# taichi-dev/taichi-nerfs

Measured on AMD Instinct MI355X. Metric: training rays/sec, higher is better.
Workload: dtype f32-table+f16-mlp

## Files before the change

taichi-nerfs_amd/csrc/mlp.hip:

```cpp
#include "ngp_device.h"
#include <stdlib.h>

namespace ngp {

typedef _Float16 half_t;
typedef half_t half8 __attribute__((ext_vector_type(8)));
typedef half_t half4 __attribute__((ext_vector_type(4)));
typedef float floatx4 __attribute__((ext_vector_type(4)));

#define NGP_MFMA(a, b, c) __builtin_amdgcn_mfma_f32_16x16x32_f16((a), (b), (c), 0, 0, 0)

constexpr int N_FWD_FRAGS = 20;
constexpr int N_ALL_FRAGS = 42;
constexpr int F_W1 = 0;
constexpr int F_W2 = 4;
constexpr int F_W3 = 6;
constexpr int F_W4 = 10;
constexpr int F_W5 = 18;
constexpr int B_W5T = 20;
constexpr int B_W4T = 24;
constexpr int B_W3T = 32;
constexpr int B_W2T = 34;
constexpr int B_W1T = 38;

__device__ __forceinline__ int chain_k(int s, int g, int j) { return 32 * s + 16 * (j >> 2) + 4 * g + (j & 3); }

__device__ __forceinline__ int pair_nat(int p, int slot) { return slot < 2 ? 2 * p + slot : 2 * (15 - p) + (slot - 2); }
__device__ __forceinline__ int enc_feat(int pairs, int g, int j) { return pairs ? pair_nat(2 * g + (j >> 2), j & 3) : 8 * g + j; }
__device__ __forceinline__ int enc_row(int pairs, int mt, int i) { return pairs ? pair_nat(4 * mt + (i >> 2), i & 3) : 16 * mt + i; }

__device__ __forceinline__ void pack_one(int tid, const float* W1, const float* W2, const float* W3, const float* W4,
                                         const float* W5, int pairs, half_t* wpack) {
    const int j = tid & 7, lane = (tid >> 3) & 63, frag = tid >> 9;
    const int i = lane & 15, g = lane >> 4;
    float v = 0.0f;
    if (frag < F_W2) {
        const int mt = frag - F_W1;
        v = W1[(16 * mt + i) * 32 + enc_feat(pairs, g, j)];
    } else if (frag < F_W3) {
        const int s = frag - F_W2;
        v = W2[i * 64 + chain_k(s, g, j)];
    } else if (frag < F_W4) {
        const int mt = frag - F_W3;
        const int k = (j < 4) ? (4 * g + j) : (16 + 4 * g + (j - 4));
        v = W3[(16 * mt + i) * 32 + k];
    } else if (frag < F_W5) {
        const int mt = (frag - F_W4) >> 1, s = (frag - F_W4) & 1;
        v = W4[(16 * mt + i) * 64 + chain_k(s, g, j)];
    } else if (frag < B_W5T) {
        const int s = frag - F_W5;
        v = (i < 3) ? W5[i * 64 + chain_k(s, g, j)] : 0.0f;
    } else if (frag < B_W4T) {
        const int mt = frag - B_W5T;
        const int k = 4 * g + j;
        v = (j < 4 && k < 3) ? W5[k * 64 + 16 * mt + i] : 0.0f;
    } else if (frag < B_W3T) {
        const int mt = (frag - B_W4T) >> 1, s = (frag - B_W4T) & 1;
        v = W4[chain_k(s, g, j) * 64 + 16 * mt + i];
    } else if (frag < B_W2T) {
        const int s = frag - B_W3T;
        v = W3[chain_k(s, g, j) * 32 + 16 + i];
    } else if (frag < B_W1T) {
        const int mt = frag - B_W2T;
        v = (j < 4) ? W2[(4 * g + j) * 64 + 16 * mt + i] : 0.0f;
    } else {
        const int mt = (frag - B_W1T) >> 1, s = (frag - B_W1T) & 1;
        v = W1[chain_k(s, g, j) * 32 + enc_row(pairs, mt, i)];
    }
    wpack[tid] = (half_t)v;
}

__global__ void __launch_bounds__(256) mlp_pack_kernel(const float* __restrict__ W1, const float* __restrict__ W2,
                                                       const float* __restrict__ W3, const float* __restrict__ W4,
                                                       const float* __restrict__ W5, int pairs, half_t* __restrict__ wpack) {
    const int tid = blockIdx.x * blockDim.x + threadIdx.x;
    if (tid < N_ALL_FRAGS * 64 * 8) pack_one(tid, W1, W2, W3, W4, W5, pairs, wpack);
}

__device__ __forceinline__ void adam_mlp_pack_block(float* __restrict__ p, float* __restrict__ g, float* __restrict__ m,
                                                    float* __restrict__ v, const float* __restrict__ sf,
                                                    const int32_t* __restrict__ si, float beta1, float beta2, float eps,
                                                    int pairs, half_t* __restrict__ wpack) {
    __shared__ float wl[9408];
    const bool skip = si[SI_SKIP] != 0;
    const AdamConsts ac = adam_consts(sf, beta1, beta2, eps);
    constexpr int PER = (9408 + 1023) / 1024;
    float pi[PER], gi[PER], mi[PER], vi[PER];
#pragma unroll
    for (int k = 0; k < PER; ++k) {
        const int i = (int)threadIdx.x + 1024 * k, ic = i < 9408 ? i : 0;
        pi[k] = p[ic]; gi[k] = g[ic]; mi[k] = m[ic]; vi[k] = v[ic];
    }
#pragma unroll
    for (int k = 0; k < PER; ++k) {
        const int i = (int)threadIdx.x + 1024 * k;
        if (i >= 9408) continue;
        if (!skip) {
            float mk = mi[k], vk = vi[k];
            adam_update(pi[k], mk, vk, gi[k], ac);
            p[i] = pi[k]; m[i] = mk; v[i] = vk;
        }
        g[i] = 0.0f;
        wl[i] = pi[k];
    }
    __syncthreads();
    for (int item = threadIdx.x; item < N_ALL_FRAGS * 64; item += blockDim.x) {
#pragma unroll
        for (int j = 0; j < 8; ++j) pack_one(8 * item + j, wl, wl + 2048, wl + 3072, wl + 5120, wl + 9216, pairs, wpack);
    }
}

__global__ void __launch_bounds__(1024) adam_mlp_pack_kernel(float* __restrict__ p, float* __restrict__ g, float* __restrict__ m,
                                                             float* __restrict__ v, const float* __restrict__ sf,
                                                             const int32_t* __restrict__ si, float beta1, float beta2, float eps,
                                                             int pairs, half_t* __restrict__ wpack) {
    adam_mlp_pack_block(p, g, m, v, sf, si, beta1, beta2, eps, pairs, wpack);
}

template <int SHADOW, bool GRAD16>
__global__ void __launch_bounds__(1024) adam_all_kernel(float4* __restrict__ tp, void* __restrict__ tg, float4* __restrict__ tm,
                                                        float4* __restrict__ tv, long n4, uint2* __restrict__ shadow,
                                                        float* __restrict__ p, float* __restrict__ g, float* __restrict__ m,
                                                        float* __restrict__ v, const float* __restrict__ sf,
                                                        const int32_t* __restrict__ si, float beta1, float beta2, float eps,
                                                        int pairs, half_t* __restrict__ wpack) {
    if (blockIdx.x == 0) { if (p) adam_mlp_pack_block(p, g, m, v, sf, si, beta1, beta2, eps, pairs, wpack); }
    else adam_table_pass<SHADOW, GRAD16>(tp, tg, tm, tv, n4, sf, si, beta1, beta2, eps, shadow, (long)blockIdx.x - 1, (long)gridDim.x - 1);
}

typedef unsigned short ushort4v __attribute__((ext_vector_type(4)));
__device__ __forceinline__ half4 to_h4(const floatx4& d) { return __builtin_convertvector(d, half4); }
__device__ __forceinline__ half4 relu_h4(const floatx4& d) {
    const half4 z = {(half_t)0, (half_t)0, (half_t)0, (half_t)0};
    return __builtin_elementwise_max(to_h4(d), z);
}
__device__ __forceinline__ half8 cat_h4(const half4& a, const half4& b) {
    return __builtin_shufflevector(a, b, 0, 1, 2, 3, 4, 5, 6, 7);
}
__device__ __forceinline__ half4 mask_h4(const floatx4& d, const half4& act) {
    typedef unsigned int uint2v __attribute__((ext_vector_type(2)));
    const uint2v a = __builtin_bit_cast(uint2v, act), h = __builtin_bit_cast(uint2v, to_h4(d));
    uint2v r;
    asm("v_pk_sub_i16 %0, 0, %2\n\t"
        "v_pk_sub_i16 %1, 0, %3\n\t"
        "v_pk_ashrrev_i16 %0, 15, %0 op_sel_hi:[0,1]\n\t"
        "v_pk_ashrrev_i16 %1, 15, %1 op_sel_hi:[0,1]\n\t"
        "v_and_b32 %0, %0, %4\n\t"
        "v_and_b32 %1, %1, %5"
        : "=&v"(r.x), "=&v"(r.y) : "v"(a.x), "v"(a.y), "v"(h.x), "v"(h.y));
    return __builtin_bit_cast(half4, r);
}

__device__ __forceinline__ float fast_exp(float x) { return __expf(x); }
__device__ __forceinline__ float fast_rcp(float x) { return __builtin_amdgcn_rcpf(x); }
__device__ __forceinline__ float fast_rsq(float x) { return __builtin_amdgcn_rsqf(x); }

__device__ __forceinline__ half4 sh_quad(int g, float x, float y, float z) {
    const float xy = x * y, xz = x * z, yz = y * z, x2 = x * x, y2 = y * y, z2 = z * z;
    float a, b, c, d;
    if (g == 0) {
        a = 0.28209479177387814f; b = -0.48860251190291987f * y; c = 0.48860251190291987f * z; d = -0.48860251190291987f * x;
    } else if (g == 1) {
        a = 1.0925484305920792f * xy; b = -1.0925484305920792f * yz; c = 0.94617469575755997f * z2 - 0.31539156525251999f;
        d = -1.0925484305920792f * xz;
    } else if (g == 2) {
        a = 0.54627421529603959f * x2 - 0.54627421529603959f * y2; b = 0.59004358992664352f * y * (-3.0f * x2 + y2);
        c = 2.8906114426405538f * xy * z; d = 0.45704579946446572f * y * (1.0f - 5.0f * z2);
    } else {
        a = 0.3731763325901154f * z * (5.0f * z2 - 3.0f); b = 0.45704579946446572f * x * (1.0f - 5.0f * z2);
        c = 1.4453057213202769f * z * (x2 - y2); d = 0.59004358992664352f * x * (-x2 + 3.0f * y2);
    }
    half4 r;
    r[0] = (half_t)a; r[1] = (half_t)b; r[2] = (half_t)c; r[3] = (half_t)d;
    return r;
}

__device__ __forceinline__ half4 sh_quad_flat(int g, float x, float y, float z) {
    const float xy = x * y, xz = x * z, yz = y * z, x2 = x * x, y2 = y * y, z2 = z * z;
    const float a0 = 0.28209479177387814f, b0 = -0.48860251190291987f * y, c0 = 0.48860251190291987f * z, d0 = -0.48860251190291987f * x;
    const float a1 = 1.0925484305920792f * xy, b1 = -1.0925484305920792f * yz, c1 = 0.94617469575755997f * z2 - 0.31539156525251999f,
                d1 = -1.0925484305920792f * xz;
    const float a2 = 0.54627421529603959f * x2 - 0.54627421529603959f * y2, b2 = 0.59004358992664352f * y * (-3.0f * x2 + y2),
                c2 = 2.8906114426405538f * xy * z, d2 = 0.45704579946446572f * y * (1.0f - 5.0f * z2);
    const float a3 = 0.3731763325901154f * z * (5.0f * z2 - 3.0f), b3 = 0.45704579946446572f * x * (1.0f - 5.0f * z2),
                c3 = 1.4453057213202769f * z * (x2 - y2), d3 = 0.59004358992664352f * x * (-x2 + 3.0f * y2);
    const bool g0 = g == 0, g1 = g == 1, g2 = g == 2;
    half4 r;
    r[0] = (half_t)(g0 ? a0 : (g1 ? a1 : (g2 ? a2 : a3)));
    r[1] = (half_t)(g0 ? b0 : (g1 ? b1 : (g2 ? b2 : b3)));
    r[2] = (half_t)(g0 ? c0 : (g1 ? c1 : (g2 ? c2 : c3)));
    r[3] = (half_t)(g0 ? d0 : (g1 ? d1 : (g2 ? d2 : d3)));
    return r;
}

__device__ __forceinline__ void enc_ptrs(const float* __restrict__ enc, int pairs, size_t plane, int smp, int g, const float*& p0,
                                         const float*& p1) {
    if (pairs) { p0 = enc + ((size_t)(2 * g) * plane + smp) * 4; p1 = enc + ((size_t)(2 * g + 1) * plane + smp) * 4; }
    else { p0 = enc + (size_t)smp * 32 + 8 * g; p1 = p0 + 4; }
}

struct TileFwd {
    half8 b_enc;
    half4 a1[4];
    half4 h;
    half8 b_in3;
    half4 a3[4], a4[4];
    half4 rgb;
    float sigma;
};

__device__ __forceinline__ const half8& wfrag(const half8* __restrict__ wl, int id, int lane) { return wl[id * 64 + lane]; }

template <bool COLOR, bool FLAT_SH = false, class WF>
__device__ __forceinline__ void tile_forward_frags(const WF& W, int g, const float4& e0, const float4& e1,
                                                   float dx, float dy, float dz, TileFwd& t) {
    const floatx4 zero = {0.f, 0.f, 0.f, 0.f};
    t.b_enc[0] = (half_t)e0.x; t.b_enc[1] = (half_t)e0.y; t.b_enc[2] = (half_t)e0.z; t.b_enc[3] = (half_t)e0.w;
    t.b_enc[4] = (half_t)e1.x; t.b_enc[5] = (half_t)e1.y; t.b_enc[6] = (half_t)e1.z; t.b_enc[7] = (half_t)e1.w;
#pragma unroll
    for (int mt = 0; mt < 4; ++mt) t.a1[mt] = relu_h4(NGP_MFMA(W(F_W1 + mt), t.b_enc, zero));
    floatx4 d2 = NGP_MFMA(W(F_W2 + 0), cat_h4(t.a1[0], t.a1[1]), zero);
    d2 = NGP_MFMA(W(F_W2 + 1), cat_h4(t.a1[2], t.a1[3]), d2);
    t.h = to_h4(d2);
    t.sigma = expf((float)t.h[0]);
    if (!COLOR) return;
    const float inv = fast_rsq(dx * dx + dy * dy + dz * dz);
    const float x = (dx * inv + 1.0f) / 2.0f, y = (dy * inv + 1.0f) / 2.0f, z = (dz * inv + 1.0f) / 2.0f;
    t.b_in3 = cat_h4(FLAT_SH ? sh_quad_flat(g, x, y, z) : sh_quad(g, x, y, z), t.h);
    const float nan_dir = 0.0f * (x + y + z);
#pragma unroll
    for (int mt = 0; mt < 4; ++mt) t.a3[mt] = relu_h4(NGP_MFMA(W(F_W3 + mt), t.b_in3, zero));
    const half8 b30 = cat_h4(t.a3[0], t.a3[1]), b31 = cat_h4(t.a3[2], t.a3[3]);
#pragma unroll
    for (int mt = 0; mt < 4; ++mt) {
        floatx4 d4 = NGP_MFMA(W(F_W4 + 2 * mt), b30, zero);
        d4 = NGP_MFMA(W(F_W4 + 2 * mt + 1), b31, d4);
        t.a4[mt] = relu_h4(d4);
    }
    floatx4 d5 = NGP_MFMA(W(F_W5 + 0), cat_h4(t.a4[0], t.a4[1]), zero);
    d5 = NGP_MFMA(W(F_W5 + 1), cat_h4(t.a4[2], t.a4[3]), d5);
#pragma unroll
    for (int r = 0; r < 4; ++r) {
        const float c = (float)(half_t)d5[r] + nan_dir;
        t.rgb[r] = (half_t)fast_rcp(1.0f + fast_exp(-c));
    }
}

template <bool COLOR>
__device__ __forceinline__ void tile_forward_regs(const half8* __restrict__ wl, int lane, int g, const float4& e0, const float4& e1,
                                                  float dx, float dy, float dz, TileFwd& t) {
    tile_forward_frags<COLOR>([&](int id) -> const half8& { return wl[id * 64 + lane]; }, g, e0, e1, dx, dy, dz, t);
}

template <int THREADS, int N_FRAGS>
__device__ __forceinline__ void load_wpack(const half_t* __restrict__ wpack, half8* __restrict__ wl) {
    const uint4* src = reinterpret_cast<const uint4*>(wpack);
    uint4* dst = reinterpret_cast<uint4*>(wl);
    constexpr int PER = (N_FRAGS * 64 + THREADS - 1) / THREADS;
    uint4 v[PER];
#pragma unroll
    for (int i = 0; i < PER; ++i) {
        const int k = threadIdx.x + i * THREADS;
        v[i] = src[k < N_FRAGS * 64 ? k : 0];
    }
#pragma unroll
    for (int i = 0; i < PER; ++i) {
        const int k = threadIdx.x + i * THREADS;
        if (k < N_FRAGS * 64) dst[k] = v[i];
    }
    __syncthreads();
}

struct FwdIn { float4 e0, e1; float dx, dy, dz; };
template <bool COLOR, bool PAIRS>
__device__ __forceinline__ void fwd_request(FwdIn& raw, const float* __restrict__ enc, const float* __restrict__ dirs, int smp, int S,
                                            int g, size_t plane) {
    const size_t s0 = smp < S ? (size_t)smp : 0;
    const float *ep0, *ep1;
    enc_ptrs(enc, PAIRS ? 1 : 0, plane, (int)s0, g, ep0, ep1);
    raw.e0 = *reinterpret_cast<const float4*>(ep0);
// ... 213 lines not shown
            floatx4 dh = NGP_MFMA(wfrag(wl, B_W3T + 0, lane), cat_h4(dz3[0], dz3[1]), zero);
            dh = NGP_MFMA(wfrag(wl, B_W3T + 1, lane), cat_h4(dz3[2], dz3[3]), dh);
            dz2 = to_h4(dh);
            if (g == 0) {
                const float h0 = (float)t.h[0];
                const half_t gs = (half_t)(in.dsig * fast_exp(fminf(fmaxf(h0, -15.0f), 15.0f)));
                dz2[0] = (half_t)((float)dz2[0] + (float)gs);
            }
            __builtin_amdgcn_sched_barrier(0);
            const half8 b_dz2 = cat_h4(dz2, hzero);
#pragma unroll
            for (int mt = 0; mt < 4; ++mt) dz1[mt] = mask_h4(NGP_MFMA(wfrag(wl, B_W2T + mt, lane), b_dz2, zero), t.a1[mt]);
            __builtin_amdgcn_sched_barrier(0);
            const half8 b10 = cat_h4(dz1[0], dz1[1]), b11 = cat_h4(dz1[2], dz1[3]);
#pragma unroll
            for (int mt = 0; mt < 2; ++mt) {
                floatx4 d = NGP_MFMA(wfrag(wl, B_W1T + 2 * mt, lane), b10, zero);
                d = NGP_MFMA(wfrag(wl, B_W1T + 2 * mt + 1, lane), b11, d);
                bad_denc |= !(isfinite(d[0]) && isfinite(d[1]) && isfinite(d[2]) && isfinite(d[3]));
                if (smp < S) {
                    float* dp = pairs ? d_enc + ((size_t)(4 * mt + g) * plane + smp) * 4 : d_enc + (size_t)smp * 32 + 16 * mt + 4 * g;
                    *reinterpret_cast<float4*>(dp) = make_float4(d[0], d[1], d[2], d[3]);
                }
                __builtin_amdgcn_sched_barrier(0);
            }
        }

        MLP_T(2);
        bwd_request(raw, enc, dirs, dsigmas, drgbs, src_next, g, pairs, plane);
        img_store(img, A_DZ5, lofs, dz5);
#pragma unroll
        for (int mt = 0; mt < 4; ++mt) {
            img_store(img, A_DZ4 + mt, lofs, dz4[mt]);
            img_store(img, A_A4 + mt, lofs, t.a4[mt]);
            img_store(img, A_A3 + mt, lofs, t.a3[mt]);
        }
        __syncthreads();
        if (lo8) {
#pragma unroll 3
            for (int k = 0; k < BG; ++k) {
                const half_t* Ik = Iall + k * IMG_HALFS;
                const half8 a = img_load_tr(Ik, A_DZ4 + mtL, g, n);
                accA0 = NGP_MFMA(a, img_load_tr(Ik, A_A3 + 2 * ntL, g, n), accA0);
                accA1 = NGP_MFMA(a, img_load_tr(Ik, A_A3 + 2 * ntL + 1, g, n), accA1);
            }
        } else {
#pragma unroll 3
            for (int k = 0; k < BG; ++k) {
                const half_t* Ik = Iall + k * IMG_HALFS;
                accC = NGP_MFMA(img_load_tr(Ik, A_DZ5, g, n), img_load_tr(Ik, A_A4 + v4, g, n), accC);
            }
        }
        __syncthreads();
        MLP_T(3);
        img_store(img, B_DZ2, lofs, dz2);
        img_store(img, B_IN3, lofs, __builtin_shufflevector(t.b_in3, t.b_in3, 0, 1, 2, 3));
        img_store(img, B_IN3 + 1, lofs, __builtin_shufflevector(t.b_in3, t.b_in3, 4, 5, 6, 7));
#pragma unroll
        for (int mt = 0; mt < 4; ++mt) {
            img_store(img, B_DZ3 + mt, lofs, dz3[mt]);
            img_store(img, B_A1 + mt, lofs, t.a1[mt]);
        }
        __syncthreads();
        if (lo8) {
#pragma unroll 3
            for (int k = 0; k < BG; ++k) {
                const half_t* Ik = Iall + k * IMG_HALFS;
                accB = NGP_MFMA(img_load_tr(Ik, B_DZ3 + mtL, g, n), img_load_tr(Ik, B_IN3 + ntL, g, n), accB);
            }
        } else {
#pragma unroll 3
            for (int k = 0; k < BG; ++k) {
                const half_t* Ik = Iall + k * IMG_HALFS;
                accB = NGP_MFMA(img_load_tr(Ik, B_DZ2, g, n), img_load_tr(Ik, B_A1 + v4, g, n), accB);
            }
        }
        __syncthreads();
        MLP_T(4);
#pragma unroll
        for (int mt = 0; mt < 4; ++mt) img_store(img, C_DZ1 + mt, lofs, dz1[mt]);
        {
            const int te = C_ENC + (g >> 1), sw = n >> 2, gi = 2 * (g & 1);
            img_store(img, te, lrow + 4 * (gi ^ sw), __builtin_shufflevector(t.b_enc, t.b_enc, 0, 1, 2, 3));
            img_store(img, te, lrow + 4 * ((gi + 1) ^ sw), __builtin_shufflevector(t.b_enc, t.b_enc, 4, 5, 6, 7));
        }
        __syncthreads();
        if (lo8) {
#pragma unroll 3
            for (int k = 0; k < BG; ++k) {
                const half_t* Ik = Iall + k * IMG_HALFS;
                accC = NGP_MFMA(img_load_tr(Ik, C_DZ1 + mtL, g, n), img_load_tr(Ik, C_ENC + ntL, g, n), accC);
            }
        }
        __syncthreads();
        MLP_T(5);
    }

    if (!dW && !parts) { if (found_inf && bad_denc) *found_inf = 1; return; }
    bool bad = false;
    float* slab = parts ? parts + (size_t)blockIdx.x * N_W : nullptr;
    auto leave = [&](int w, float v) {
        if (slab) slab[w] = v;
        else if (v != 0.0f) unsafeAtomicAdd(dW + w, v);
    };
#pragma unroll
    for (int r = 0; r < 4; ++r) {
        const int o = 16 * mtL + 4 * g + r, o2 = 4 * g + r;
        const float a0 = accA0[r], a1 = accA1[r], b = accB[r], c = accC[r];
        if (lo8) {
            leave(OFF_W4 + o * 64 + 32 * ntL + n, a0);
            leave(OFF_W4 + o * 64 + 32 * ntL + 16 + n, a1);
            leave(OFF_W3 + o * 32 + 16 * ntL + n, b);
            leave(OFF_W1 + o * 32 + enc_feat(pairs, (16 * ntL + n) >> 3, n & 7), c);
        } else {
            leave(OFF_W2 + o2 * 64 + 16 * v4 + n, b);
            if (o2 < 3) leave(OFF_W5 + o2 * 64 + 16 * v4 + n, c);
        }
        bad |= !isfinite(a0) || !isfinite(a1) || !isfinite(b) || !isfinite(c);
    }
    if (found_inf && (bad || bad_denc)) *found_inf = 1;
}

#ifdef NGP_MLP_BWD_REG
#include "../../profiles/microbench/mlp_bwd_reg_kernel.inc"
#endif

}

using namespace ngp;

extern "C" {

#ifdef NGP_MLP_DIAG
int ngp_mlp_debug_read(unsigned long long* host128, int reset) {
    if (hipMemcpyFromSymbol(host128, HIP_SYMBOL(ngp_mlp_dbg), sizeof(ngp_mlp_dbg)) != hipSuccess) return -1;
    if (reset) { unsigned long long z[16 * 8] = {}; if (hipMemcpyToSymbol(HIP_SYMBOL(ngp_mlp_dbg), z, sizeof(z)) != hipSuccess) return -1; }
    return 0;
}
#endif

int ngp_mlp_wpack_halfs(void) { return N_ALL_FRAGS * 64 * 8; }

int ngp_mlp_pack(const float* W1, const float* W2, const float* W3, const float* W4, const float* W5, int enc_pairs, uint16_t* wpack,
                 void* stream) {
    const int total = N_ALL_FRAGS * 64 * 8;
    hipLaunchKernelGGL(mlp_pack_kernel, dim3((total + 255) / 256), dim3(256), 0, (hipStream_t)stream, W1, W2, W3, W4, W5, enc_pairs,
                       (half_t*)wpack);
    NGP_LAUNCH_CHECK();
    return 0;
}

int ngp_adam_mlp_pack(float* p, float* g, float* m, float* v, const float* state_f, const int32_t* state_i, float beta1, float beta2,
                      float eps, int enc_pairs, uint16_t* wpack, void* stream) {
    hipLaunchKernelGGL(adam_mlp_pack_kernel, dim3(1), dim3(1024), 0, (hipStream_t)stream, p, g, m, v, state_f, state_i, beta1, beta2,
                       eps, enc_pairs, (half_t*)wpack);
    NGP_LAUNCH_CHECK();
    return 0;
}

#define NGP_ADAM_ALL(SH, G16)                                                                                                     \
    hipLaunchKernelGGL((adam_all_kernel<SH, G16>), grid, block, 0, (hipStream_t)stream, (float4*)table, table_g, (float4*)table_m,    \
                       (float4*)table_v, n4, (uint2*)table_16, mlp, mlp_g, mlp_m, mlp_v, state_f, state_i, beta1, beta2, eps,         \
                       enc_pairs, (half_t*)wpack)

int ngp_adam_all_ex(float* table, void* table_g, int grad_is_f16, float* table_m, float* table_v, long long n, uint16_t* table_16,
                    int copy_kind, float* mlp, float* mlp_g, float* mlp_m, float* mlp_v, const float* state_f, const int32_t* state_i,
                    float beta1, float beta2, float eps, int enc_pairs, uint16_t* wpack, void* stream) {
    if (n <= 0 || n % 4 != 0) return -1;
    if ((copy_kind != 0) != (table_16 != nullptr) || copy_kind < 0 || copy_kind > 2) return -1;
    const long n4 = (long)(n / 4);
    long blocks = (n4 + 1023) / 1024;
    if (blocks > 256L * 4) blocks = 256L * 4;
    const dim3 grid((unsigned)blocks + 1), block(1024);
    if (grad_is_f16) {
        if (copy_kind == 2) NGP_ADAM_ALL(2, true); else if (copy_kind == 1) NGP_ADAM_ALL(1, true); else NGP_ADAM_ALL(0, true);
    } else {
        if (copy_kind == 2) NGP_ADAM_ALL(2, false); else if (copy_kind == 1) NGP_ADAM_ALL(1, false); else NGP_ADAM_ALL(0, false);
    }
    NGP_LAUNCH_CHECK();
    return 0;
}
#undef NGP_ADAM_ALL

int ngp_adam_all(float* table, float* table_g, float* table_m, float* table_v, long long n, uint16_t* table_bf16, float* mlp,
                 float* mlp_g, float* mlp_m, float* mlp_v, const float* state_f, const int32_t* state_i, float beta1, float beta2,
                 float eps, int enc_pairs, uint16_t* wpack, void* stream) {
    return ngp_adam_all_ex(table, table_g, 0, table_m, table_v, n, table_bf16, table_bf16 ? 1 : 0, mlp, mlp_g, mlp_m, mlp_v, state_f,
                           state_i, beta1, beta2, eps, enc_pairs, wpack, stream);
}

static inline int mlp_grid(int S) {
    static const int cap = [] { const char* e = ngp_experiment("mlp_fwd_blocks"); const int v = e ? atoi(e) : 0; return v > 0 ? v : 768; }();
    const int iters = (S + 31) / 32;
    int blocks = (iters + 3) / 4;
    if (blocks > cap) blocks = cap;
    return blocks < 1 ? 1 : blocks;
}

int ngp_mlp_fwd_ex(const float* enc, const float* dirs, const uint16_t* wpack, int n_max, const int32_t* n_dev, int enc_pairs,
                   float* sigmas, uint16_t* rgbs, void* stream) {
    if (n_max <= 0) return 0;
#define NGP_FWD(C, P, D, R)                                                                                          \
    hipLaunchKernelGGL((mlp_fwd_kernel<C, P>), dim3(mlp_grid(n_max)), dim3(256), 0, (hipStream_t)stream, enc, (const float*)(D), \
                       (const half_t*)wpack, n_max, n_dev, sigmas, (half_t*)(R))
    if (dirs && rgbs) { if (enc_pairs) NGP_FWD(true, true, dirs, rgbs); else NGP_FWD(true, false, dirs, rgbs); }
    else { if (enc_pairs) NGP_FWD(false, true, nullptr, nullptr); else NGP_FWD(false, false, nullptr, nullptr); }
#undef NGP_FWD
    NGP_LAUNCH_CHECK();
    return 0;
}

int ngp_mlp_fwd_list(const float* enc, const float* dirs, const uint16_t* wpack, int n_max, const int32_t* n_list, const int32_t* list,
                     int enc_pairs, float* sigmas, uint16_t* rgbs, void* stream) {
    if (n_max <= 0) return 0;
    if (!n_list || !list || !dirs || !rgbs) return -1;
    if (enc_pairs) hipLaunchKernelGGL((mlp_fwd_kernel<true, true, true>), dim3(mlp_grid(n_max)), dim3(256), 0, (hipStream_t)stream, enc, dirs,
                                      (const half_t*)wpack, n_max, n_list, sigmas, (half_t*)rgbs, list);
    else hipLaunchKernelGGL((mlp_fwd_kernel<true, false, true>), dim3(mlp_grid(n_max)), dim3(256), 0, (hipStream_t)stream, enc, dirs,
                            (const half_t*)wpack, n_max, n_list, sigmas, (half_t*)rgbs, list);
    NGP_LAUNCH_CHECK();
    return 0;
}

int ngp_mlp_fwd(const float* enc, const float* dirs, const uint16_t* wpack, int n, float* sigmas, uint16_t* rgbs, void* stream) {
    return ngp_mlp_fwd_ex(enc, dirs, wpack, n, nullptr, 0, sigmas, rgbs, stream);
}

static int mlp_bwd_launch(const float* enc, const float* dirs, const uint16_t* wpack, const float* dsigmas, const uint16_t* drgbs,
                          int n_max, const int32_t* n_dev, const int32_t* live_idx, int enc_pairs, float* d_enc, float* dW,
                          float* parts, int32_t* found_inf, void* stream) {
    int blocks;
#ifdef NGP_MLP_BWD_REG
    const char* form = ngp_experiment("mlp_bwd");
    if (form && form[0] == 'r') {
        if ((long long)n_max * 128 > 0xffffffffLL) return -1;
        blocks = ((n_max + 31) / 32 + RW - 1) / RW;
        if (blocks > 256) blocks = 256;
        if (blocks < 1) blocks = 1;
#define NGP_BWD_REG(P, L)                                                                                                        \
    hipLaunchKernelGGL((mlp_bwd_reg_kernel<P, L>), dim3(blocks), dim3(64 * RW), 0, (hipStream_t)stream, enc, dirs, (const half_t*)wpack, \
                       dsigmas, (const half_t*)drgbs, n_max, n_dev, live_idx, d_enc, dW, parts, found_inf)
        if (enc_pairs) { if (live_idx) NGP_BWD_REG(true, true); else NGP_BWD_REG(true, false); }
        else { if (live_idx) NGP_BWD_REG(false, true); else NGP_BWD_REG(false, false); }
#undef NGP_BWD_REG
        NGP_LAUNCH_CHECK();
        return blocks;
    }
#endif
    blocks = ((n_max + 31) / 32 + BG - 1) / BG;
    if (blocks > 256) blocks = 256;
    if (blocks < 1) blocks = 1;
    hipLaunchKernelGGL(mlp_bwd_kernel, dim3(blocks), dim3(64 * BW), 0, (hipStream_t)stream, enc, dirs, (const half_t*)wpack, dsigmas,
                       (const half_t*)drgbs, n_max, n_dev, live_idx, enc_pairs, d_enc, dW, parts, found_inf);
    NGP_LAUNCH_CHECK();
    return blocks;
}

int ngp_mlp_bwd_live(const float* enc, const float* dirs, const uint16_t* wpack, const float* dsigmas, const uint16_t* drgbs,
                     int n_max, const int32_t* n_dev, const int32_t* live_idx, int enc_pairs, float* d_enc, float* dW,
                     int32_t* found_inf, void* stream) {
    if (n_max <= 0) return 0;
    const int rc = mlp_bwd_launch(enc, dirs, wpack, dsigmas, drgbs, n_max, n_dev, live_idx, enc_pairs, d_enc, dW, nullptr, found_inf,
                                  stream);
    return rc < 0 ? rc : 0;
}

int ngp_mlp_dw_parts_max(void) { return 256; }

int ngp_mlp_bwd_live_parts(const float* enc, const float* dirs, const uint16_t* wpack, const float* dsigmas, const uint16_t* drgbs,
                           int n_max, const int32_t* n_dev, const int32_t* live_idx, int enc_pairs, float* d_enc, float* dW_parts,
                           int32_t* found_inf, void* stream) {
    if (n_max <= 0) return 0;
    if (!dW_parts) return -1;
    return mlp_bwd_launch(enc, dirs, wpack, dsigmas, drgbs, n_max, n_dev, live_idx, enc_pairs, d_enc, nullptr, dW_parts, found_inf,
                          stream);
}

__global__ void __launch_bounds__(NGP_MLP_REDUCE_THREADS) mlp_dw_reduce_kernel(const float* __restrict__ parts, int n_parts, float* __restrict__ dW) {
    mlp_dw_reduce_block(parts, n_parts, dW, blockIdx.x);
}

int ngp_mlp_dw_reduce(const float* dW_parts, int n_parts, float* dW, void* stream) {
    if (n_parts <= 0) return 0;
    hipLaunchKernelGGL(mlp_dw_reduce_kernel, dim3(NGP_MLP_REDUCE_BLOCKS), dim3(NGP_MLP_REDUCE_THREADS), 0, (hipStream_t)stream, dW_parts, n_parts, dW);
    NGP_LAUNCH_CHECK();
    return 0;
}

int ngp_mlp_bwd_ex(const float* enc, const float* dirs, const uint16_t* wpack, const float* dsigmas, const uint16_t* drgbs,
                   int n_max, const int32_t* n_dev, int enc_pairs, float* d_enc, float* dW, int32_t* found_inf, void* stream) {
    return ngp_mlp_bwd_live(enc, dirs, wpack, dsigmas, drgbs, n_max, n_dev, nullptr, enc_pairs, d_enc, dW, found_inf, stream);
}

int ngp_mlp_bwd(const float* enc, const float* dirs, const uint16_t* wpack, const float* dsigmas, const uint16_t* drgbs, int n,
                float* d_enc, float* dW, void* stream) {
    return ngp_mlp_bwd_ex(enc, dirs, wpack, dsigmas, drgbs, n, nullptr, 0, d_enc, dW, nullptr, stream);
}

}
```

taichi-nerfs_amd/ngp_hip/lib.py:

```python
import ctypes
import os
import shutil
import subprocess

_HERE = os.path.dirname(os.path.abspath(__file__))
PKG_ROOT = os.path.dirname(_HERE)
CSRC = os.path.join(PKG_ROOT, "csrc")
INCLUDE = os.path.join(os.path.dirname(PKG_ROOT), "include")
LIB_PATH = os.path.join(CSRC, "libngp_hip.so")
SOURCES = ["march.hip", "hash_grid.hip", "hash_bwd_lds.hip", "composite.hip", "sh_grid.hip", "mlp.hip", "optim.hip", "distortion.hip", "occupancy.hip", "rays.hip",
           "render.hip", "exchange.hip", "triplane.hip", "voxel_grid.hip", "deploy.hip"]
HEADERS = ["ngp_device.h", "hash_common.h"]
HIPCC_FLAGS = ["--offload-arch=gfx950", "-O3", "-std=c++17", "-ffp-contract=off", "-fPIC", "-shared"]
FLAGS_STAMP = LIB_PATH + ".flags"

NGP_MAX_LEVELS = 16


class HashLevels(ctypes.Structure):
    _fields_ = [
        ("n_levels", ctypes.c_int32),
        ("n_features", ctypes.c_int32),
        ("begin_fast_hash_level", ctypes.c_int32),
        ("total_entries", ctypes.c_int32),
        ("scale", ctypes.c_float * NGP_MAX_LEVELS),
        ("resolution", ctypes.c_uint32 * NGP_MAX_LEVELS),
        ("map_size", ctypes.c_uint32 * NGP_MAX_LEVELS),
        ("offset", ctypes.c_uint32 * NGP_MAX_LEVELS),
        ("bwd_plan", ctypes.c_uint32),
    ]

    def with_plan(self, bits):
        bits = int(bits)
        if bits == self.bwd_plan:
            return self
        cache = self.__dict__.setdefault("_plans", {})
        lv = cache.get(bits)
        if lv is None:
            lv = HashLevels()
            ctypes.memmove(ctypes.byref(lv), ctypes.byref(self), ctypes.sizeof(HashLevels))
            lv.bwd_plan = bits
            cache[bits] = lv
        return lv


BWD_PLAN_DETERMINISTIC, BWD_PLAN_CONCENTRATED = 1, 2


class TriPlaneLevels(ctypes.Structure):
    _fields_ = [
        ("n_levels", ctypes.c_int32),
        ("n_features", ctypes.c_int32),
        ("max_res", ctypes.c_int32),
        ("reserved", ctypes.c_int32),
        ("scale", ctypes.c_float * NGP_MAX_LEVELS),
        ("resolution", ctypes.c_uint32 * NGP_MAX_LEVELS),
    ]


def _render_fields():
    P, I, F, LL = ctypes.c_void_p, ctypes.c_int32, ctypes.c_float, ctypes.c_longlong
    ptrs = lambda *names: [(k, P) for k in names]
    return (ptrs("rays_o", "rays_d", "hits_t", "noise") + [("n_rays", I), ("max_samples", I)]
            + ptrs("bitfield", "coarse") + [("rebuild_coarse", I), ("cascades", I), ("grid_size", I)]
            + [("scale", F), ("exp_step_factor", F), ("T_threshold", F)]
            + [("table", P), ("table_kind", I), ("enc_pairs", I), ("levels", P), ("lo", F), ("hi", F)]
            + [("w", P * 5), ("wpack", P), ("cap", LL)]
            + ptrs("stage", "march_ctr", "xyzs", "dirs", "deltas", "ts", "enc", "sigmas", "rgbs", "ws")
            + ptrs("rays_a", "total", "vr_per_ray", "opacity", "depth", "rgb")
            + ptrs("g_opacity", "g_depth", "g_rgb", "g_ws")
            + ptrs("d_sigmas", "d_rgbs", "d_enc", "live_off", "live_idx", "live_total")
            + [("workspace", P), ("workspace_bytes", LL), ("force_atomic", I), ("reserved", I)]
            + ptrs("dW_parts", "live_zero")
            + [("dW", P), ("dtable", P), ("dtable_bytes", LL)]
            + [("bg", F), ("clear_grads", I), ("rgb_out", P)])


class RenderArgs(ctypes.Structure):
    _fields_ = _render_fields()


def _sources():
    return [os.path.join(CSRC, s) for s in SOURCES if os.path.exists(os.path.join(CSRC, s))]


def _flags():
    return HIPCC_FLAGS + os.environ.get("NGP_HIPCC_EXTRA", "").split()


def needs_build():
    if not os.path.exists(LIB_PATH):
        return True
    t = os.path.getmtime(LIB_PATH)
    deps = _sources() + [os.path.join(CSRC, h) for h in HEADERS] + [os.path.join(INCLUDE, "ngp_hip.h"), os.path.join(INCLUDE, "ngp_hip_experimental.h")]
    if any(os.path.getmtime(d) > t for d in deps if os.path.exists(d)):
        return True
    if os.path.exists(FLAGS_STAMP):
        return open(FLAGS_STAMP).read().split() != _flags()
    return bool(os.environ.get("NGP_HIPCC_EXTRA", "").split())


def build(force=False, verbose=False):
    if not force and not needs_build():
        return LIB_PATH
    hipcc = shutil.which("hipcc") or "/opt/rocm/bin/hipcc"
    if not os.path.exists(hipcc):
        raise RuntimeError("hipcc not found: cannot build libngp_hip.so")
    tmp = LIB_PATH + ".tmp.%d" % os.getpid()
    cmd = [hipcc] + _flags() + ["-o", tmp] + _sources()
    if verbose:
        print(" ".join(cmd))
    res = subprocess.run(cmd, capture_output=True, text=True)
    if res.returncode != 0:
        raise RuntimeError("hipcc failed:\n" + res.stdout + res.stderr)
    os.replace(tmp, LIB_PATH)
    with open(FLAGS_STAMP, "w") as f:
        f.write(" ".join(_flags()))
    return LIB_PATH


_P = ctypes.c_void_p
_I = ctypes.c_int
_F = ctypes.c_float
_LV = ctypes.POINTER(HashLevels)
_TLV = ctypes.POINTER(TriPlaneLevels)

SIGNATURES = {
    "ngp_abi_version": [],
    "ngp_hash_levels_init": [_LV, ctypes.c_double, _I, ctypes.c_double, ctypes.c_double, _I],
    "ngp_ray_aabb": [_P, _P, _F, _I, _P, _P],
    "ngp_march_train_count": [_P, _P, _P, _P, _P, _I, _I, _F, _F, _I, _I, _P, _P, _P],
    "ngp_bitfield_coarsen": [_P, _I, _I, _P, _P],
    "ngp_march_train_count_ex": [_P, _P, _P, _P, _P, _P, _I, _I, _F, _F, _I, _I, _P, _P, _P],
    "ngp_march_train_scan": [_P, _I, _P, _P, _P],
    "ngp_march_train_fused": [_P, _P, _P, _P, _P, _P, _I, _I, _F, _F, _I, _I, _P, _P, _P, _P, _P, _P, _P, _P, _P],
    "ngp_march_train_fused_cap": [_P, _P, _P, _P, _P, _P, _I, _I, _F, _F, _I, _I, ctypes.c_longlong, _P, _P, _P, _P, _P, _P, _P, _P, _P],
    "ngp_march_train_fused_rng": [_P, _P, _P, _P, _P, ctypes.c_ulonglong, _I, _I, _F, _F, _I, _I, _P, _P, _P, _P, _P, _P, _P, _P, _P],
    "ngp_march_train_fused_shaped": [_P, _P, _P, _P, _P, _P, ctypes.c_ulonglong, _I, _I, _F, _F, _I, _I, _I, _I, _P, _P, _P, _P, _P, _P, _P,
                                     _P, _P],
    "ngp_rng_uniform": [ctypes.c_ulonglong, _I, _P, _P],
    "ngp_hash_fwd_list": [_P, _P, _I, _LV, _I, _P, _P, _I, _F, _F, _I, _P, _P],
    "ngp_mlp_fwd_list": [_P, _P, _P, _I, _P, _P, _I, _P, _P, _P],
    "ngp_live_list": [_P, _P, _I, _P, _P, _P, _P],
    "ngp_mse_loss_grad_rays": [_P, _P, _P, _F, _I, _P, _P, _P, _P, _P],
    "ngp_chunk_schedule": [_P, _P, _P, _I, _I, _I, _I, _F, _P, _P, _P, _P, _P],
    "ngp_march_train_write": [_P, _P, _P, _P, _I, _I, _P, _P, _P, _P, _P],
    "ngp_march_test": [_P, _P, _P, _P, _P, _I, _I, _F, _F, _I, _I, _P, _P, _P, _P, _P, _P],
    "ngp_hash_fwd_f32": [_P, _P, _LV, _I, _P, _P],
    "ngp_hash_bwd_f32": [_P, _P, _LV, _I, _P, _P],
    "ngp_hash_fwd_f32_ex": [_P, _P, _LV, _I, _P, _I, _F, _F, _I, _P, _P],
    "ngp_hash_fwd_bf16_ex": [_P, _P, _LV, _I, _P, _I, _F, _F, _I, _P, _P],
    "ngp_hash_bwd_f32_ex": [_P, _P, _LV, _I, _P, _I, _F, _F, _I, _P, _P, _P],
    "ngp_hash_fwd_f16": [_P, _P, _LV, _I, _P, _P],
    "ngp_hash_bwd_f16": [_P, _P, _LV, _I, _P, _P],
    "ngp_hash_fwd_f16_ex": [_P, _P, _LV, _I, _P, _I, _F, _F, _I, _P, _P],
    "ngp_hash_bwd_f16_ex": [_P, _P, _LV, _I, _P, _I, _F, _F, _I, _P, _P, _P],
    "ngp_check_finite_f16": [_P, ctypes.c_longlong, _P, _P],
    "ngp_live_compact": [_P, _P, _I, _P, _P, _P, _P],
    "ngp_mlp_bwd_live": [_P, _P, _P, _P, _P, _I, _P, _P, _I, _P, _P, _P, _P],
    "ngp_mlp_dw_parts_max": [],
    "ngp_mlp_bwd_live_parts": [_P, _P, _P, _P, _P, _I, _P, _P, _I, _P, _P, _P, _P],
    "ngp_mlp_dw_reduce": [_P, _I, _P, _P],
    "ngp_hash_bwd_f32_live": [_P, _P, _LV, _I, _P, _P, _I, _F, _F, _I, _P, _P, _P],
    "ngp_hash_bwd_f16_live": [_P, _P, _LV, _I, _P, _P, _I, _F, _F, _I, _P, _P, _P],
    "ngp_hash_bwd_sliced_workspace": [_LV, _I],
# ... 115 lines not shown
```

Baseline: 17.91 million.

## Spread MLP Adam+pack over multiple blocks via compile-time inverse slot map

Replaces the single-block MLP Adam update and fragment packing, which staged the weights in LDS, with a per-weight scatter. A constexpr inverse map gives each weight up to two packed fp16 slots, so the work spreads across ten 1024-thread blocks in the fused optimizer kernel and across many 256-thread blocks in the standalone kernel. This removes the serial single-block tail on the optimizer's critical path. In exchange it adds a large constexpr table in device memory and a slower compile-time evaluation, and unused padding slots in wpack are no longer written with zeros.

Result: faster. 18.30 million, median of 5 (+2.2%).

```diff
diff --git a/taichi-nerfs_amd/csrc/mlp.hip b/taichi-nerfs_amd/csrc/mlp.hip
--- a/taichi-nerfs_amd/csrc/mlp.hip
+++ b/taichi-nerfs_amd/csrc/mlp.hip
@@ -1,4 +1,5 @@
 #include "ngp_device.h"
+#include "mlp_slot_map.h"
 #include <stdlib.h>
 
 namespace ngp {
@@ -10,63 +11,16 @@
 
 #define NGP_MFMA(a, b, c) __builtin_amdgcn_mfma_f32_16x16x32_f16((a), (b), (c), 0, 0, 0)
 
-constexpr int N_FWD_FRAGS = 20;
-constexpr int N_ALL_FRAGS = 42;
-constexpr int F_W1 = 0;
-constexpr int F_W2 = 4;
-constexpr int F_W3 = 6;
-constexpr int F_W4 = 10;
-constexpr int F_W5 = 18;
-constexpr int B_W5T = 20;
-constexpr int B_W4T = 24;
-constexpr int B_W3T = 32;
-constexpr int B_W2T = 34;
-constexpr int B_W1T = 38;
-
-__device__ __forceinline__ int chain_k(int s, int g, int j) { return 32 * s + 16 * (j >> 2) + 4 * g + (j & 3); }
-
-__device__ __forceinline__ int pair_nat(int p, int slot) { return slot < 2 ? 2 * p + slot : 2 * (15 - p) + (slot - 2); }
-__device__ __forceinline__ int enc_feat(int pairs, int g, int j) { return pairs ? pair_nat(2 * g + (j >> 2), j & 3) : 8 * g + j; }
-__device__ __forceinline__ int enc_row(int pairs, int mt, int i) { return pairs ? pair_nat(4 * mt + (i >> 2), i & 3) : 16 * mt + i; }
 
 __device__ __forceinline__ void pack_one(int tid, const float* W1, const float* W2, const float* W3, const float* W4,
                                          const float* W5, int pairs, half_t* wpack) {
-    const int j = tid & 7, lane = (tid >> 3) & 63, frag = tid >> 9;
-    const int i = lane & 15, g = lane >> 4;
+    const int idx = mlp_slot_source(tid, pairs);
     float v = 0.0f;
-    if (frag < F_W2) {
-        const int mt = frag - F_W1;
-        v = W1[(16 * mt + i) * 32 + enc_feat(pairs, g, j)];
-    } else if (frag < F_W3) {
-        const int s = frag - F_W2;
-        v = W2[i * 64 + chain_k(s, g, j)];
-    } else if (frag < F_W4) {
-        const int mt = frag - F_W3;
-        const int k = (j < 4) ? (4 * g + j) : (16 + 4 * g + (j - 4));
-        v = W3[(16 * mt + i) * 32 + k];
-    } else if (frag < F_W5) {
-        const int mt = (frag - F_W4) >> 1, s = (frag - F_W4) & 1;
-        v = W4[(16 * mt + i) * 64 + chain_k(s, g, j)];
-    } else if (frag < B_W5T) {
-        const int s = frag - F_W5;
-        v = (i < 3) ? W5[i * 64 + chain_k(s, g, j)] : 0.0f;
-    } else if (frag < B_W4T) {
-        const int mt = frag - B_W5T;
-        const int k = 4 * g + j;
-        v = (j < 4 && k < 3) ? W5[k * 64 + 16 * mt + i] : 0.0f;
-    } else if (frag < B_W3T) {
-        const int mt = (frag - B_W4T) >> 1, s = (frag - B_W4T) & 1;
-        v = W4[chain_k(s, g, j) * 64 + 16 * mt + i];
-    } else if (frag < B_W2T) {
-        const int s = frag - B_W3T;
-        v = W3[chain_k(s, g, j) * 32 + 16 + i];
-    } else if (frag < B_W1T) {
-        const int mt = frag - B_W2T;
-        v = (j < 4) ? W2[(4 * g + j) * 64 + 16 * mt + i] : 0.0f;
-    } else {
-        const int mt = (frag - B_W1T) >> 1, s = (frag - B_W1T) & 1;
-        v = W1[chain_k(s, g, j) * 32 + enc_row(pairs, mt, i)];
-    }
+    if (idx >= MLP_OFF_W5) v = W5[idx - MLP_OFF_W5];
+    else if (idx >= MLP_OFF_W4) v = W4[idx - MLP_OFF_W4];
+    else if (idx >= MLP_OFF_W3) v = W3[idx - MLP_OFF_W3];
+    else if (idx >= MLP_OFF_W2) v = W2[idx - MLP_OFF_W2];
+    else if (idx >= 0) v = W1[idx];
     wpack[tid] = (half_t)v;
 }
 
@@ -77,55 +31,60 @@
     if (tid < N_ALL_FRAGS * 64 * 8) pack_one(tid, W1, W2, W3, W4, W5, pairs, wpack);
 }
 
-__device__ __forceinline__ void adam_mlp_pack_block(float* __restrict__ p, float* __restrict__ g, float* __restrict__ m,
-                                                    float* __restrict__ v, const float* __restrict__ sf,
-                                                    const int32_t* __restrict__ si, float beta1, float beta2, float eps,
-                                                    int pairs, half_t* __restrict__ wpack) {
-    __shared__ float wl[9408];
-    const bool skip = si[SI_SKIP] != 0;
-    const AdamConsts ac = adam_consts(sf, beta1, beta2, eps);
-    constexpr int PER = (9408 + 1023) / 1024;
-    float pi[PER], gi[PER], mi[PER], vi[PER];
-#pragma unroll
-    for (int k = 0; k < PER; ++k) {
-        const int i = (int)threadIdx.x + 1024 * k, ic = i < 9408 ? i : 0;
-        pi[k] = p[ic]; gi[k] = g[ic]; mi[k] = m[ic]; vi[k] = v[ic];
-    }
-#pragma unroll
-    for (int k = 0; k < PER; ++k) {
-        const int i = (int)threadIdx.x + 1024 * k;
-        if (i >= 9408) continue;
-        if (!skip) {
-            float mk = mi[k], vk = vi[k];
-            adam_update(pi[k], mk, vk, gi[k], ac);
-            p[i] = pi[k]; m[i] = mk; v[i] = vk;
-        }
-        g[i] = 0.0f;
-        wl[i] = pi[k];
-    }
-    __syncthreads();
-    for (int item = threadIdx.x; item < N_ALL_FRAGS * 64; item += blockDim.x) {
-#pragma unroll
-        for (int j = 0; j < 8; ++j) pack_one(8 * item + j, wl, wl + 2048, wl + 3072, wl + 5120, wl + 9216, pairs, wpack);
-    }
-}
-
-__global__ void __launch_bounds__(1024) adam_mlp_pack_kernel(float* __restrict__ p, float* __restrict__ g, float* __restrict__ m,
-                                                             float* __restrict__ v, const float* __restrict__ sf,
-                                                             const int32_t* __restrict__ si, float beta1, float beta2, float eps,
-                                                             int pairs, half_t* __restrict__ wpack) {
-    adam_mlp_pack_block(p, g, m, v, sf, si, beta1, beta2, eps, pairs, wpack);
+constexpr MlpSlotInverse mlp_slot_inverse_host[2] = {mlp_slot_inverse(0), mlp_slot_inverse(1)};
+__device__ const MlpSlotInverse mlp_slot_inverse_dev[2] = {mlp_slot_inverse_host[0], mlp_slot_inverse_host[1]};
+static_assert(MLP_SLOT_FANOUT == 2 && sizeof(mlp_slot_inverse_host[0].slot[0]) == sizeof(uint32_t), "a weight's slot list is one 32-bit load");
+static_assert(MLP_WEIGHTS == NGP_MLP_NW, "the optimizer and the weight-gradient reduction agree on the weight count");
+static inline bool mlp_slot_inverse_ok() {
+    return mlp_slot_inverse_host[0].max_fanout <= MLP_SLOT_FANOUT && mlp_slot_inverse_host[1].max_fanout <= MLP_SLOT_FANOUT &&
+           mlp_slot_inverse_host[0].bad_source == 0 && mlp_slot_inverse_host[1].bad_source == 0;
+}
+
+constexpr int ADAM_ALL_THREADS = 1024;
+constexpr int ADAM_ALL_MLP_BLOCKS = (MLP_WEIGHTS + ADAM_ALL_THREADS - 1) / ADAM_ALL_THREADS;
+constexpr int ADAM_MLP_THREADS = 256;
+
+__device__ __forceinline__ void adam_mlp_pack_weight(int i, float* __restrict__ p, float* __restrict__ g, float* __restrict__ m,
+                                                     float* __restrict__ v, const float* __restrict__ sf,
+                                                     const int32_t* __restrict__ si, float beta1, float beta2, float eps,
+                                                     int pairs, half_t* __restrict__ wpack) {
+    if (i >= MLP_WEIGHTS) return;
+    const uint32_t slots = reinterpret_cast<const uint32_t*>(mlp_slot_inverse_dev[pairs ? 1 : 0].slot)[i];
+    float pi = p[i], mi = m[i], vi = v[i];
+    const float gi = g[i];
+    if (si[SI_SKIP] == 0) {
+        const AdamConsts ac = adam_consts(sf, beta1, beta2, eps);
+        adam_update(pi, mi, vi, gi, ac);
+        p[i] = pi; m[i] = mi; v[i] = vi;
+    }
+    g[i] = 0.0f;
+    const uint16_t h = (uint16_t)f16_bits_rn(pi);
+    uint16_t* __restrict__ w16 = reinterpret_cast<uint16_t*>(wpack);
+    const uint32_t s0 = slots & 0xffffu, s1 = slots >> 16;
+    if (s0 != MLP_NO_SLOT) w16[s0] = h;
+    if (s1 != MLP_NO_SLOT) w16[s1] = h;
+}
+
+__global__ void __launch_bounds__(ADAM_MLP_THREADS) adam_mlp_pack_kernel(float* __restrict__ p, float* __restrict__ g,
+                                                                         float* __restrict__ m, float* __restrict__ v,
+                                                                         const float* __restrict__ sf, const int32_t* __restrict__ si,
+                                                                         float beta1, float beta2, float eps, int pairs,
+                                                                         half_t* __restrict__ wpack) {
+    adam_mlp_pack_weight((int)(blockIdx.x * blockDim.x + threadIdx.x), p, g, m, v, sf, si, beta1, beta2, eps, pairs, wpack);
 }
 
 template <int SHADOW, bool GRAD16>
-__global__ void __launch_bounds__(1024) adam_all_kernel(float4* __restrict__ tp, void* __restrict__ tg, float4* __restrict__ tm,
+__global__ void __launch_bounds__(ADAM_ALL_THREADS) adam_all_kernel(float4* __restrict__ tp, void* __restrict__ tg, float4* __restrict__ tm,
                                                         float4* __restrict__ tv, long n4, uint2* __restrict__ shadow,
                                                         float* __restrict__ p, float* __restrict__ g, float* __restrict__ m,
                                                         float* __restrict__ v, const float* __restrict__ sf,
                                                         const int32_t* __restrict__ si, float beta1, float beta2, float eps,
                                                         int pairs, half_t* __restrict__ wpack) {
-    if (blockIdx.x == 0) { if (p) adam_mlp_pack_block(p, g, m, v, sf, si, beta1, beta2, eps, pairs, wpack); }
-    else adam_table_pass<SHADOW, GRAD16>(tp, tg, tm, tv, n4, sf, si, beta1, beta2, eps, shadow, (long)blockIdx.x - 1, (long)gridDim.x - 1);
+    const int k = p ? ADAM_ALL_MLP_BLOCKS : 0;
+    if ((int)blockIdx.x < k)
+        adam_mlp_pack_weight((int)(blockIdx.x * ADAM_ALL_THREADS + threadIdx.x), p, g, m, v, sf, si, beta1, beta2, eps, pairs, wpack);
+    else
+        adam_table_pass<SHADOW, GRAD16>(tp, tg, tm, tv, n4, sf, si, beta1, beta2, eps, shadow, (long)blockIdx.x - k, (long)gridDim.x - k);
 }
 
 typedef unsigned short ushort4v __attribute__((ext_vector_type(4)));
@@ -645,8 +604,9 @@
 
 int ngp_adam_mlp_pack(float* p, float* g, float* m, float* v, const float* state_f, const int32_t* state_i, float beta1, float beta2,
                       float eps, int enc_pairs, uint16_t* wpack, void* stream) {
-    hipLaunchKernelGGL(adam_mlp_pack_kernel, dim3(1), dim3(1024), 0, (hipStream_t)stream, p, g, m, v, state_f, state_i, beta1, beta2,
-                       eps, enc_pairs, (half_t*)wpack);
+    if (!mlp_slot_inverse_ok()) return -1;
+    hipLaunchKernelGGL(adam_mlp_pack_kernel, dim3((MLP_WEIGHTS + ADAM_MLP_THREADS - 1) / ADAM_MLP_THREADS), dim3(ADAM_MLP_THREADS), 0,
+                       (hipStream_t)stream, p, g, m, v, state_f, state_i, beta1, beta2, eps, enc_pairs, (half_t*)wpack);
     NGP_LAUNCH_CHECK();
     return 0;
 }
@@ -664,7 +624,8 @@
     const long n4 = (long)(n / 4);
     long blocks = (n4 + 1023) / 1024;
     if (blocks > 256L * 4) blocks = 256L * 4;
-    const dim3 grid((unsigned)blocks + 1), block(1024);
+    if (mlp && !mlp_slot_inverse_ok()) return -1;
+    const dim3 grid((unsigned)blocks + (mlp ? ADAM_ALL_MLP_BLOCKS : 0)), block(ADAM_ALL_THREADS);
     if (grad_is_f16) {
         if (copy_kind == 2) NGP_ADAM_ALL(2, true); else if (copy_kind == 1) NGP_ADAM_ALL(1, true); else NGP_ADAM_ALL(0, true);
     } else {
diff --git a/taichi-nerfs_amd/csrc/mlp_slot_map.h b/taichi-nerfs_amd/csrc/mlp_slot_map.h
--- /dev/null
+++ b/taichi-nerfs_amd/csrc/mlp_slot_map.h
@@ -0,0 +1,103 @@
+#pragma once
+#include <stdint.h>
+
+#if defined(__HIPCC__) || defined(__CUDACC__)
+#define NGP_HD __host__ __device__
+#else
+#define NGP_HD
+#endif
+
+namespace ngp {
+
+constexpr int N_FWD_FRAGS = 20;
+constexpr int N_ALL_FRAGS = 42;
+constexpr int MLP_SLOTS = N_ALL_FRAGS * 64 * 8;
+constexpr int MLP_WEIGHTS = 9408;
+constexpr int MLP_OFF_W1 = 0, MLP_OFF_W2 = 2048, MLP_OFF_W3 = 3072, MLP_OFF_W4 = 5120, MLP_OFF_W5 = 9216;
+constexpr int F_W1 = 0;
+constexpr int F_W2 = 4;
+constexpr int F_W3 = 6;
+constexpr int F_W4 = 10;
+constexpr int F_W5 = 18;
+constexpr int B_W5T = 20;
+constexpr int B_W4T = 24;
+constexpr int B_W3T = 32;
+constexpr int B_W2T = 34;
+constexpr int B_W1T = 38;
+
+NGP_HD constexpr int chain_k(int s, int g, int j) { return 32 * s + 16 * (j >> 2) + 4 * g + (j & 3); }
+
+NGP_HD constexpr int pair_nat(int p, int slot) { return slot < 2 ? 2 * p + slot : 2 * (15 - p) + (slot - 2); }
+NGP_HD constexpr int enc_feat(int pairs, int g, int j) { return pairs ? pair_nat(2 * g + (j >> 2), j & 3) : 8 * g + j; }
+NGP_HD constexpr int enc_row(int pairs, int mt, int i) { return pairs ? pair_nat(4 * mt + (i >> 2), i & 3) : 16 * mt + i; }
+
+NGP_HD constexpr int mlp_slot_source(int tid, int pairs) {
+    const int j = tid & 7, lane = (tid >> 3) & 63, frag = tid >> 9;
+    const int i = lane & 15, g = lane >> 4;
+    if (frag < F_W2) {
+        const int mt = frag - F_W1;
+        return MLP_OFF_W1 + (16 * mt + i) * 32 + enc_feat(pairs, g, j);
+    } else if (frag < F_W3) {
+        const int s = frag - F_W2;
+        return MLP_OFF_W2 + i * 64 + chain_k(s, g, j);
+    } else if (frag < F_W4) {
+        const int mt = frag - F_W3;
+        const int k = (j < 4) ? (4 * g + j) : (16 + 4 * g + (j - 4));
+        return MLP_OFF_W3 + (16 * mt + i) * 32 + k;
+    } else if (frag < F_W5) {
+        const int mt = (frag - F_W4) >> 1, s = (frag - F_W4) & 1;
+        return MLP_OFF_W4 + (16 * mt + i) * 64 + chain_k(s, g, j);
+    } else if (frag < B_W5T) {
+        const int s = frag - F_W5;
+        return (i < 3) ? MLP_OFF_W5 + i * 64 + chain_k(s, g, j) : -1;
+    } else if (frag < B_W4T) {
+        const int mt = frag - B_W5T;
+        const int k = 4 * g + j;
+        return (j < 4 && k < 3) ? MLP_OFF_W5 + k * 64 + 16 * mt + i : -1;
+    } else if (frag < B_W3T) {
+        const int mt = (frag - B_W4T) >> 1, s = (frag - B_W4T) & 1;
+        return MLP_OFF_W4 + chain_k(s, g, j) * 64 + 16 * mt + i;
+    } else if (frag < B_W2T) {
+        const int s = frag - B_W3T;
+        return MLP_OFF_W3 + chain_k(s, g, j) * 32 + 16 + i;
+    } else if (frag < B_W1T) {
+        const int mt = frag - B_W2T;
+        return (j < 4) ? MLP_OFF_W2 + (4 * g + j) * 64 + 16 * mt + i : -1;
+    } else {
+        const int mt = (frag - B_W1T) >> 1, s = (frag - B_W1T) & 1;
+        return MLP_OFF_W1 + chain_k(s, g, j) * 32 + enc_row(pairs, mt, i);
+    }
+}
+
+constexpr int MLP_SLOT_FANOUT = 2;
+constexpr uint16_t MLP_NO_SLOT = 0xffffu;
+static_assert(MLP_SLOTS < MLP_NO_SLOT, "slot numbers are stored in 16 bits");
+
+struct MlpSlotInverse {
+    uint16_t slot[MLP_WEIGHTS][MLP_SLOT_FANOUT];
+    int max_fanout;
+    int bad_source;
+};
+
+constexpr void mlp_slot_inverse_frag(MlpSlotInverse& inv, uint8_t* count, int frag, int pairs) {
+    for (int tid = frag * 512; tid < (frag + 1) * 512; ++tid) {
+        const int w = mlp_slot_source(tid, pairs);
+        if (w == -1) continue;
+        if (w < -1 || w >= MLP_WEIGHTS) { ++inv.bad_source; continue; }
+        if (count[w] < MLP_SLOT_FANOUT) inv.slot[w][count[w]] = (uint16_t)tid;
+        if (count[w] < 255) ++count[w];
+    }
+}
+
+constexpr MlpSlotInverse mlp_slot_inverse(int pairs) {
+    MlpSlotInverse inv = {};
+    uint8_t count[MLP_WEIGHTS] = {};
+    for (int w = 0; w < MLP_WEIGHTS; ++w)
+        for (int k = 0; k < MLP_SLOT_FANOUT; ++k) inv.slot[w][k] = MLP_NO_SLOT;
+    for (int frag = 0; frag < N_ALL_FRAGS; ++frag) mlp_slot_inverse_frag(inv, count, frag, pairs);
+    for (int w = 0; w < MLP_WEIGHTS; ++w)
+        if (count[w] > inv.max_fanout) inv.max_fanout = count[w];
+    return inv;
+}
+
+}
diff --git a/taichi-nerfs_amd/ngp_hip/lib.py b/taichi-nerfs_amd/ngp_hip/lib.py
--- a/taichi-nerfs_amd/ngp_hip/lib.py
+++ b/taichi-nerfs_amd/ngp_hip/lib.py
@@ -10,7 +10,7 @@
 LIB_PATH = os.path.join(CSRC, "libngp_hip.so")
 SOURCES = ["march.hip", "hash_grid.hip", "hash_bwd_lds.hip", "composite.hip", "sh_grid.hip", "mlp.hip", "optim.hip", "distortion.hip", "occupancy.hip", "rays.hip",
            "render.hip", "exchange.hip", "triplane.hip", "voxel_grid.hip", "deploy.hip"]
-HEADERS = ["ngp_device.h", "hash_common.h"]
+HEADERS = ["ngp_device.h", "hash_common.h", "mlp_slot_map.h"]
 HIPCC_FLAGS = ["--offload-arch=gfx950", "-O3", "-std=c++17", "-ffp-contract=off", "-fPIC", "-shared"]
 FLAGS_STAMP = LIB_PATH + ".flags"
 
```
